# bio-phys/BioEM

Measured on AMD Instinct MI355X. Metric: image-comparisons/sec (orient×CTF×particle) at 224²; log P max-abs-diff vs CPU, higher is better.
Workload: dtype f32

## Files before the change

### bioem_amd/csrc/bioem_hip.hip

```cpp
#define BIOEM_MAIN_TU 1
#include "engine_types.hpp"

#include <rccl/rccl.h>

#include <dlfcn.h>

#include <map>
#include <memory>
#include <mutex>
#include <queue>
#include <string>
#include <vector>

namespace
{

struct HipErr
{
  std::string msg;
};

#define HIP_CHECK(h, expr)                                                                                         \
  do                                                                                                               \
  {                                                                                                                \
// ... 21 lines not shown
#include "compare_generic.hpp"
#include "compare_rows.hpp"
#include "compare_direct.hpp"
#include "kernel_select.hpp"
#include "fold_kernels.hpp"
#include "window_tiles.hpp"

struct bioem_hip_ctx
{
  int device = 0;
  hipStream_t stream = nullptr;
  PD pd;
  int nMaps = 0, nAngles = 0, nCTF = 0, algo = 1;
  int N = 0, H = 0, M = 0;
  int Hp = 0;
  size_t Mc = 0;
  KernelPlan plan;
  int pchunk = 128;
  int *dDispLocal = nullptr, *dTileCenter = nullptr, *dTileValid = nullptr, *dRankOfRow = nullptr;
  float *dBtab = nullptr;
  float2 *dConvShift = nullptr;
  Partial *dPartTiles = nullptr;
  int OB = 0;
  int maxOC = 0;
  int chunkB = 0;

  float2 *dRef = nullptr;
  float *dSumRef = nullptr, *dSumsqRef = nullptr;
  float2 *dCTF = nullptr;
  float *dCtfParam = nullptr;
  bioem_hip_model_point *dPts = nullptr;
  double *dStamp = nullptr;
  double modelRadius = 0.;
  double quatNormDev = 0.;
  int nPts = 0;
  float NormDen = 0, pixelSize = 0;
  int shiftX = 0, shiftY = 0;
  int iradMax = 0;
  bool direct = false;
  float *dMapsReal = nullptr, *dConvReal = nullptr;
  double2 *dDirectZ = nullptr;
  int nCU = 256;
  float4 *dAngles = nullptr;
  int nAnglesUp = 0, isQuat = 1;
  float2 *dTw = nullptr;
  double2 *dTwD = nullptr;
  int *dDisp = nullptr;
  double2 *dLtab = nullptr;
  float2 *dTwk = nullptr;
  float2 *dTwNyq = nullptr;
  float *dTnyq = nullptr;
  Partial *dPartials = nullptr;
  unsigned char *dProb = nullptr;
  size_t probBytes = 0;
  size_t devProbBytes = 0;
  bool shard = false;
  int angO0 = 0, angO1 = 0;
  bioem_hip_angle_candidate *dCand = nullptr;
  int candK = 0;
  unsigned char *dSend = nullptr, *dRecv = nullptr;
  size_t sendBytes = 0, recvBytes = 0;
  bioem_hip_prob_map *dMerged = nullptr;

  struct Slot
  {
    double *projReal = nullptr;
    double *tempDen = nullptr;
    double2 *rowSpec = nullptr;
    float2 *specRef = nullptr;
    float *scratch = nullptr;
    float2 *conv = nullptr;
    bioem_hip_param5 *params = nullptr;
    double2 *postc = nullptr;
    int stageO0 = 0, stageNO = 0, stageC0 = 0, stageNC = 0;
    hipEvent_t prepDone = nullptr, cmpDone = nullptr;
    bool cmpPending = false;
  };
  Slot slot[2];
  hipStream_t prepStream = nullptr;

  struct CompatHalf
  {
    float2 *hConv = nullptr;
    bioem_hip_param5 *hPar = nullptr;
    int2 *hIds = nullptr;
    int4 *hSeg = nullptr;
    float2 *dStage = nullptr;
    int2 *dIds = nullptr;
    int4 *dSeg = nullptr;
    hipEvent_t staged = nullptr;
  };
  CompatHalf ring[2];
  int ringCap = 0, ringHalf = 0, ringCount = 0;
  std::vector<int> ringOrients;
  hipStream_t copyStream = nullptr;

  struct Alloc
  {
    void *p;
    bool pinned;
  };
  std::vector<Alloc> allocs;

  struct PhaseEvents
  {
    int phase, o0, o1, c0, c1;
    hipEvent_t a, b;
  };
  bool phaseTiming = false;
  std::vector<PhaseEvents> phasePending;
  std::vector<bioem_hip_phase_record> phaseDone;
  std::vector<hipEvent_t> evPool;
  std::vector<std::pair<hipEvent_t, hipEvent_t>> evPending;
  double compareMs = 0;
  long long launches = 0, comparisons = 0;

  std::string err;
};

namespace
{

hipEvent_t get_event(bioem_hip_ctx *h)
{
  if (!h->evPool.empty())
  {
    hipEvent_t e = h->evPool.back();
    h->evPool.pop_back();
    return e;
  }
  hipEvent_t e;
  if (hipEventCreate(&e) != hipSuccess)
    return nullptr;
  return e;
}

void drain_events(bioem_hip_ctx *h)
{
  for (auto &pr : h->evPending)
  {
    float ms = 0.f;
    if (hipEventSynchronize(pr.second) == hipSuccess && hipEventElapsedTime(&ms, pr.first, pr.second) == hipSuccess)
      h->compareMs += (double) ms;
    h->evPool.push_back(pr.first);
    h->evPool.push_back(pr.second);
  }
  h->evPending.clear();
}

int phase_begin(bioem_hip_ctx *h, hipStream_t st, int phase, int o0, int o1, int c0, int c1)
{
  if (!h->phaseTiming)
    return 0;
  bioem_hip_ctx::PhaseEvents e = {phase, o0, o1, c0, c1, get_event(h), get_event(h)};
  if (!e.a || !e.b)
  {
    h->err = "hipEventCreate failed";
    return 1;
  }
  HIP_CHECK(h, hipEventRecord(e.a, st));
  h->phasePending.push_back(e);
  return 0;
}

int phase_end(bioem_hip_ctx *h, hipStream_t st)
{
  if (!h->phaseTiming || h->phasePending.empty())
    return 0;
  HIP_CHECK(h, hipEventRecord(h->phasePending.back().b, st));
  return 0;
}

void drain_phases(bioem_hip_ctx *h)
{
  for (auto &e : h->phasePending)
  {
    float ms = 0.f;
    if (hipEventSynchronize(e.b) == hipSuccess && hipEventElapsedTime(&ms, e.a, e.b) == hipSuccess)
    {
      bioem_hip_phase_record r = {e.phase, e.o0, e.o1, e.c0, e.c1, (double) ms * 1e-3};
      h->phaseDone.push_back(r);
    }
    h->evPool.push_back(e.a);
    h->evPool.push_back(e.b);
  }
  h->phasePending.clear();
}

template <class T>
int dev_alloc(bioem_hip_ctx *h, T *&p, size_t n)
{
  HIP_CHECK(h, hipMalloc(&p, sizeof(T) * n));
  if (p)
    h->allocs.push_back({p, false});
  return 0;
}
template <class T>
int host_alloc(bioem_hip_ctx *h, T *&p, size_t n)
{
  HIP_CHECK(h, hipHostMalloc(&p, sizeof(T) * n, hipHostMallocDefault));
  if (p)
    h->allocs.push_back({p, true});
  return 0;
}
template <class T>
void dev_release(bioem_hip_ctx *h, T *&p)
{
  if (!p)
    return;
  for (size_t i = 0; i < h->allocs.size(); i++)
    if (h->allocs[i].p == p)
    {
      h->allocs.erase(h->allocs.begin() + i);
      break;
    }
  hipFree(p);
  p = nullptr;
}
template <class T>
int upload(bioem_hip_ctx *h, T *&p, const T *src, size_t n)
{
  if (dev_alloc(h, p, n))
    return 1;
  HIP_CHECK(h, hipMemcpy(p, src, sizeof(T) * n, hipMemcpyHostToDevice));
  return 0;
}

double2 twiddle_d(long long ab, int N)
{
  const double ang = 2.0 * M_PI * (double) ((ab % N + N) % N) / (double) N;
  return make_double2(cos(ang), sin(ang));
}
float2 twiddle(long long ab, int N)
{
  const double2 w = twiddle_d(ab, N);
  return make_float2((float) w.x, (float) w.y);
}

void void_slot(bioem_hip_ctx::Slot &s) { s.stageNO = s.stageNC = 0; }

template <int Q>
void launch_nyquist_rows(bioem_hip_ctx *h, const CompareArgs &aw, int WD, int nOC)
{
  const int PB = 16 / Q;
  const dim3 gridq((unsigned) (((size_t) (h->nMaps + PB - 1) / PB) * ((nOC + 15) / 16)));
  switch (WD)
  {
#define X(W)                                                                                                            \
  case W:                                                                                                               \
    hipLaunchKernelGGL((k_nyquist_rows<W, Q>), gridq, dim3(256), 0, h->stream, aw);                                     \
    break;
    X(5) X(10) X(13) X(15) X(20) X(31) X(42)
#undef X
  }
}
void launch_nyquist(bioem_hip_ctx *h, const CompareArgs &aw, int WD, int nOC)
{
  if (h->nMaps <= 64)
    launch_nyquist_rows<4>(h, aw, WD, nOC);
  else
    launch_nyquist_rows<1>(h, aw, WD, nOC);
}

int launch_compare_fold(bioem_hip_ctx *h, const bioem_hip_ctx::Slot &bb, int nOC, int orient0, int conv0,
                        int convPerOrient, const int2 *ids = nullptr, const int4 *segs = nullptr, int nSeg = 0)
{
  const KernelPlan &P = h->plan;
  const int fam = P.family;
  CompareArgs a;
  a.ref = h->dRef;
  a.conv = bb.conv;
  a.params = bb.params;
  a.postc = bb.postc;
  a.sumRef = h->dSumRef;
  a.sumsqRef = h->dSumsqRef;
  a.tw = h->dTw;
  a.disp = h->dDisp;
  a.ltab = h->dLtab;
  a.twk = h->dTwk;
  a.btab = h->dBtab;
  a.tnyq = h->dTnyq;
  a.twnyq = h->dTwNyq;
  a.partials = h->dPartials;
  a.ldPart = h->maxOC;
  a.N = h->N;
  a.H = h->H;
  a.Hp = h->Hp;
  a.N1 = P.N1;
  a.nd = P.nd;
  a.maxD = h->pd.maxDisplaceCenter;
  a.nOC = nOC;
  a.nMaps = h->nMaps;
  a.algo = h->algo;
  a.pd = h->pd;
  a.gs = P.gs;
  a.ndx = a.ndy = P.nd;
  a.nyqWD = P.nyqWD;
  {
    const int cols = P.nyq ? h->H - 1 : h->H;
    const int nblkF = (cols + 63) / 64, rem = cols - (nblkF - 1) * 64;
    a.split = (fam == KF_FAST || fam == KF_FASTM) && rem <= 32 && P.N1 >= 2 &&
              (P.nyq || !getenv("BIOEM_NO_SPLIT_LAST"));
  }
  a.pchunk = h->pchunk > 0 ? std::min(h->pchunk, h->nMaps) : h->nMaps;
  if (a.pchunk >= 8)
    a.pchunk &= ~7;
  const int ocGroups = (nOC + 3) / 4;
  const bool groupPerXcd = h->nMaps <= 64 && (fam == KF_FAST || fam == KF_FASTM || fam == KF_FASTM2);
  if (groupPerXcd)
    a.pchunk = -1;
  dim3 grid((unsigned) ((size_t) (groupPerXcd ? (ocGroups + 7) / 8 * 8 : ocGroups) * h->nMaps)), block(256);
  if (fam == KF_WIDE2)
  {
    a.ts = P.w2TS;
    grid = dim3((unsigned) ((size_t) nOC * h->nMaps));
    block = dim3(64 * P.w2NW);
  }
  else if (fam == KF_GENERIC)
  {
    a.ts = P.genericRows;
    grid = dim3((unsigned) ((size_t) ((nOC + P.genericWaves - 1) / P.genericWaves) * h->nMaps));
    block = dim3(64 * P.genericWaves);
  }
  auto launch = [&](const CompareArgs &aw) {
    if (P.nyq)
      launch_nyquist(h, aw, P.nyqWD, nOC);
    hipLaunchKernelGGL(P.fn, grid, block, P.ldsBytes, h->stream, aw);
  };
  hipEvent_t e0 = get_event(h), e1 = get_event(h);
  if (!e0 || !e1)
  {
    if (e0)
      h->evPool.push_back(e0);
    if (e1)
      h->evPool.push_back(e1);
    h->err = "hipEventCreate failed";
    return 1;
  }
  hipLaunchKernelGGL(k_posterior_consts, dim3((nOC + 63) / 64), dim3(64), 0, h->stream, bb.params, h->pd, bb.postc, nOC);
  HIP_CHECK(h, hipEventRecord(e0, h->stream));
  if (phase_begin(h, h->stream, BIOEM_HIP_PHASE_COMPARISON, ids ? -1 : orient0, ids ? -1 : orient0 + (nOC + convPerOrient - 1) / convPerOrient,
                  ids ? -1 : conv0, ids ? -1 : conv0 + convPerOrient))
    return 1;
  if (h->direct)
  {
    CompareArgs ad = a;
    ad.gs = h->pd.GridSpaceCenter;
    ad.maxD = h->pd.maxDisplaceCenter;
    hipLaunchKernelGGL(k_c2r_cols, dim3(h->H, nOC), dim3(128), sizeof(double2) * h->N, h->stream, bb.conv, h->N, h->H,
                       P.halfR, P.N1, h->dTwD, h->dDirectZ);
    hipLaunchKernelGGL(k_c2r_rows, dim3(h->N, nOC), dim3(128), sizeof(double2) * h->H, h->stream, h->dDirectZ, h->N,
                       h->H, h->dTwD, h->dConvReal);
    const dim3 gridd((unsigned) ((size_t) nOC * ((h->nMaps + 31) / 32)));
    hipLaunchKernelGGL((k_compare_direct<3, 8>), gridd, dim3(512), direct_lds_bytes(h->N), h->stream, ad, h->dConvReal,
                       h->dMapsReal);
  }
  else if (!P.tileT)
    launch(a);
  else
  {
    const int nT = P.tilesPerAxis;
    const size_t tileStride = (size_t) h->nMaps * h->maxOC;
    const size_t total = (size_t) nOC * h->M;
    CompareArgs at = a;
    at.disp = h->dDispLocal;
    at.nd = P.tileT;
    at.maxD = P.winD * P.gs;
    for (int tx = 0; tx < nT; tx++)
      for (int ty = 0; ty < nT; ty++)
      {
        const int sx = P.gs * P.tileCenter[tx], sy = P.gs * P.tileCenter[ty];
        if (sx == 0 && sy == 0)
          at.conv = bb.conv;
        else
        {
          hipLaunchKernelGGL(k_phase_shift, dim3(2048), dim3(256), 0, h->stream, bb.conv, h->dConvShift, total, h->N,
                             h->H, P.halfR, P.N1, sx, sy, h->dTw);
          at.conv = h->dConvShift;
        }
        at.ndx = P.tileValid[tx];
        at.ndy = P.tileValid[ty];
        at.partials = h->dPartTiles + (size_t) (tx * nT + ty) * tileStride;
        launch(at);
      }
    const long long nt = (long long) nOC * h->nMaps;
    hipLaunchKernelGGL(k_merge_tiles, dim3((unsigned) ((nt + 255) / 256)), dim3(256), 0, h->stream, h->dPartTiles,
                       nT * nT, tileStride, h->maxOC, nOC, h->nMaps, P.tileT, nT, h->dTileCenter,
                       h->pd.maxDisplaceCenter / P.gs, P.nd, h->dRankOfRow, h->dPartials);
  }
  HIP_CHECK(h, hipGetLastError());
  HIP_CHECK(h, hipEventRecord(e1, h->stream));
  h->evPending.push_back({e0, e1});
  h->launches++;
  h->comparisons += (long long) nOC * h->nMaps;
  bioem_hip_prob_map *pmap = reinterpret_cast<bioem_hip_prob_map *>(h->dProb);
  bioem_hip_prob_angle *pang = reinterpret_cast<bioem_hip_prob_angle *>(h->dProb + sizeof(bioem_hip_prob_map) * h->nMaps);
  if (h->pd.writeAngles)
  {
    const int nRuns = ids ? nSeg : (nOC + convPerOrient - 1) / convPerOrient;
    const long long nt = (long long) nRuns * h->nMaps;
    hipLaunchKernelGGL(k_fold_angles, dim3((unsigned) ((nt + 255) / 256)), dim3(256), 0, h->stream, h->dPartials,
                       h->maxOC, nOC, h->nMaps, orient0, convPerOrient, segs, nRuns, pang, h->angO0);
  }
  if (h->nMaps <= 64 && nOC >= 1024)
    hipLaunchKernelGGL(k_fold_wave<4>, dim3(h->nMaps), dim3(256), 0, h->stream, h->dPartials, h->maxOC, nOC, h->nMaps,
                       bb.params, h->dSumRef, h->dDisp, P.nd, h->pd, orient0, conv0, convPerOrient, ids, pmap);
  else
    hipLaunchKernelGGL(k_fold_wave<1>, dim3((h->nMaps + 3) / 4), dim3(256), 0, h->stream, h->dPartials, h->maxOC, nOC,
                       h->nMaps, bb.params, h->dSumRef, h->dDisp, P.nd, h->pd, orient0, conv0, convPerOrient, ids,
                       pmap);
  HIP_CHECK(h, hipGetLastError());
  if (phase_end(h, h->stream))
    return 1;
  if (h->evPending.size() > 512)
    drain_events(h);
  return 0;
}

const int kMaxPixels = 5120;
constexpr int kDftTwLds = 3072;
size_t dft_rows_lds(int N) { return sizeof(double) * ((N <= kDftTwLds ? 5 : 3) * (size_t) N + 2); }
size_t dft_cols_lds(int N) { return sizeof(double2) * (N <= kDftTwLds ? 3 : 2) * (size_t) N; }
void dft_split(int N, int &A, int &B)
{
  A = 1;
  for (int d = 1; d * d <= N; d++)
    if (N % d == 0)
      A = d;
  B = N / A;
}
bool r2c_use_fft(int N)
{
  const char *e = getenv("BIOEM_R2C");
  return bioem_r2c_fft_supported(N) && !(e && !strcmp(e, "dft"));
}
bool dft_use_mfma(int N)
{
  int A, B;
  dft_split(N, A, B);
  return dft_mfma_fits(N, A, B);
}
hipError_t dft_allow_lds(int N)
{
  hipError_t e;
  if (dft_use_mfma(N))
  {
    const void *fns[4] = {reinterpret_cast<const void *>(k_dft_rows_mfma<2>),
                          reinterpret_cast<const void *>(k_dft_rows_mfma<kDftMfmaTiles>),
                          reinterpret_cast<const void *>(k_dft_cols_mfma<2>),
                          reinterpret_cast<const void *>(k_dft_cols_mfma<kDftMfmaTiles>)};
    for (int f = 0; f < 4; f++)
    {
      e = hipFuncSetAttribute(fns[f], hipFuncAttributeMaxDynamicSharedMemorySize,
                              (int) (f < 2 ? dft_mfma_rows_lds(N) : dft_mfma_cols_lds(N)));
      if (e != hipSuccess)
        return e;
    }
    return hipSuccess;
  }
  if (N <= kDftTwLds)
  {
    e = hipFuncSetAttribute(reinterpret_cast<const void *>(k_dft_rows<true>), hipFuncAttributeMaxDynamicSharedMemorySize,
                            (int) dft_rows_lds(N));
    if (e != hipSuccess)
      return e;
    return hipFuncSetAttribute(reinterpret_cast<const void *>(k_dft_cols<true>), hipFuncAttributeMaxDynamicSharedMemorySize,
                               (int) dft_cols_lds(N));
  }
  e = hipFuncSetAttribute(reinterpret_cast<const void *>(k_dft_rows<false>), hipFuncAttributeMaxDynamicSharedMemorySize,
                          (int) dft_rows_lds(N));
  if (e != hipSuccess)
    return e;
  return hipFuncSetAttribute(reinterpret_cast<const void *>(k_dft_cols<false>), hipFuncAttributeMaxDynamicSharedMemorySize,
                             (int) dft_cols_lds(N));
}

hipError_t conv_allow_lds()
{
  const void *fns[3] = {reinterpret_cast<const void *>(k_convolve_sums<3, 6>), reinterpret_cast<const void *>(k_convolve_sums<3, 5>),
                        reinterpret_cast<const void *>(k_convolve_sums<4, 4>)};
  for (const void *f : fns)
  {
    const hipError_t e = hipFuncSetAttribute(f, hipFuncAttributeMaxDynamicSharedMemorySize, (int) conv_lanes_lds(kLaneRows));
    if (e != hipSuccess)
      return e;
  }
  return hipSuccess;
}

hipError_t launch_r2c(hipStream_t st, int nCU, const double *srcD, const float *srcF, const double *tempDen, float NormDen,
                      int N, int nImg, const double2 *tw, double2 *rowSpec, float2 *out, int lo = 0, int side = 0)
{
  side = side ? side : N;
  const int H = N / 2 + 1;
  int A, B;
  dft_split(N, A, B);
  if (r2c_use_fft(N))
    return bioem_r2c_fft_launch(st, nCU, srcD, srcF, tempDen, NormDen, N, nImg, tw, rowSpec, out, lo, side);
  if (dft_use_mfma(N))
  {
    const int perCU = std::max(1, std::min(4, (int) (160 * 1024 / (dft_mfma_cols_lds(N) + 1024))));
    const int rowUnits = ((N + 15) / 16) * nImg, colUnits = ((H + 15) / 16) * nImg;
    if (A * ((B + 15) / 16) <= 2 * kDftMfmaWaves)
    {
      hipLaunchKernelGGL(k_dft_rows_mfma<2>, dim3(std::min(rowUnits, perCU * nCU)), dim3(kDftMfmaThreads),
                         dft_mfma_rows_lds(N), st, srcD, srcF, tempDen, NormDen, N, H, A, B, nImg, tw, rowSpec);
      hipLaunchKernelGGL(k_dft_cols_mfma<2>, dim3(std::min(colUnits, perCU * nCU)), dim3(kDftMfmaThreads),
                         dft_mfma_cols_lds(N), st, rowSpec, N, H, A, B, nImg, tw, out);
    }
    else
    {
      hipLaunchKernelGGL(k_dft_rows_mfma<kDftMfmaTiles>, dim3(std::min(rowUnits, nCU)), dim3(kDftMfmaThreads),
                         dft_mfma_rows_lds(N), st, srcD, srcF, tempDen, NormDen, N, H, A, B, nImg, tw, rowSpec);
      hipLaunchKernelGGL(k_dft_cols_mfma<kDftMfmaTiles>, dim3(std::min(colUnits, nCU)), dim3(kDftMfmaThreads),
                         dft_mfma_cols_lds(N), st, rowSpec, N, H, A, B, nImg, tw, out);
    }
  }
  else if (N <= kDftTwLds)
  {
    hipLaunchKernelGGL(k_dft_rows<true>, dim3(N, nImg), dim3(128), dft_rows_lds(N), st, srcD, srcF, tempDen, NormDen, N,
                       H, A, B, tw, rowSpec);
    hipLaunchKernelGGL(k_dft_cols<true>, dim3(H, nImg), dim3(256), dft_cols_lds(N), st, rowSpec, N, H, A, B, tw, out);
  }
  else
  {
    hipLaunchKernelGGL(k_dft_rows<false>, dim3(N, nImg), dim3(128), dft_rows_lds(N), st, srcD, srcF, tempDen, NormDen, N,
                       H, A, B, tw, rowSpec);
    hipLaunchKernelGGL(k_dft_cols<false>, dim3(H, nImg), dim3(256), dft_cols_lds(N), st, rowSpec, N, H, A, B, tw, out);
  }
  return hipGetLastError();
}

int run_r2c(bioem_hip_ctx *h, const bioem_hip_ctx::Slot &bb, hipStream_t st, const double *srcD, const float *srcF, int nImg,
            int lo = 0, int side = 0)
{
  HIP_CHECK(h, launch_r2c(st, h->nCU, srcD, srcF, bb.tempDen, h->NormDen, h->N, nImg, h->dTwD, bb.rowSpec, bb.specRef, lo,
                          side));
  return 0;
}

int project_batch(bioem_hip_ctx *h, const bioem_hip_ctx::Slot &bb, hipStream_t st, int o0, int nO)
{
  const int N = h->N;
  const double reach = h->modelRadius / (double) h->pixelSize;
  const int boxLo = std::max(0, (int) std::floor(N / 2.0 + 0.5 - reach) - 1 - h->iradMax - std::max(0, std::max(h->shiftX, h->shiftY)));
  const int boxHi = std::min(N - 1, (int) std::floor(N / 2.0 + 0.5 + reach) + 1 + h->iradMax - std::min(0, std::min(h->shiftX, h->shiftY)));
  const int boxSide = boxHi - boxLo + 1;
  const bool keepLength = h->quatNormDev * 4.0 * std::max(1.0, reach) < 0.5;
  if (h->dStamp && boxSide >= 1 && (size_t) boxSide * boxSide * sizeof(double) <= 52 * 1024 && N < 32768 &&
      keepLength)
  {
    const int compact = r2c_use_fft(N);
    hipLaunchKernelGGL(k_project_box, dim3(std::min(nO, 3 * h->nCU)), dim3(256), sizeof(double) * boxSide * boxSide, st,
                       h->dPts, h->nPts, h->dAngles, o0, h->isQuat, N, h->pixelSize, h->shiftX, h->shiftY, h->iradMax,
                       h->dStamp, boxLo, boxSide, nO, compact, bb.projReal, bb.tempDen);
    HIP_CHECK(h, hipGetLastError());
    return compact ? run_r2c(h, bb, st, bb.projReal, nullptr, nO, boxLo, boxSide) : run_r2c(h, bb, st, bb.projReal, nullptr, nO);
  }
  HIP_CHECK(h, hipMemsetAsync(bb.tempDen, 0, sizeof(double) * nO, st));
  const int TR = 40960 / (8 * N);
  const bool coordsFit = (size_t) h->nPts * sizeof(ProjectRecord) <= (size_t) N * h->H * sizeof(double2);
  if (TR >= 12 && h->iradMax <= 16 && h->dStamp && N < 32768 && coordsFit)
  {
    ProjectRecord *coords = reinterpret_cast<ProjectRecord *>(bb.rowSpec);
    hipLaunchKernelGGL(k_project_coords, dim3((h->nPts + 255) / 256, nO), dim3(256), 0, st, h->dPts, h->nPts, h->dAngles,
                       o0, h->isQuat, N, h->pixelSize, h->shiftX, h->shiftY, coords);
    const int units = ((N + TR - 1) / TR) * nO;
    hipLaunchKernelGGL(k_project_bands, dim3(std::min(units, 3 * h->nCU)), dim3(256), sizeof(double) * TR * N, st, coords,
                       h->nPts, nO, N, TR, h->iradMax, h->dStamp, bb.projReal, bb.tempDen);
  }
  else
  {
    HIP_CHECK(h, hipMemsetAsync(bb.projReal, 0, sizeof(double) * (size_t) nO * N * N, st));
    hipLaunchKernelGGL(k_project, dim3((h->nPts + 255) / 256, nO), dim3(256), 0, st, h->dPts, h->nPts, h->dAngles, o0,
                       h->isQuat, N, h->pixelSize, h->shiftX, h->shiftY, bb.projReal, bb.tempDen);
  }
  HIP_CHECK(h, hipGetLastError());
  return run_r2c(h, bb, st, bb.projReal, nullptr, nO);
}

int compat_alloc(bioem_hip_ctx *h)
{
  if (h->ringCap)
    return 0;
  int cap = 128;
  if (getenv("BIOEM_COMPAT_RING"))
    cap = atoi(getenv("BIOEM_COMPAT_RING"));
  cap = std::max(1, std::min(cap, h->maxOC));
  const size_t M = (size_t) h->M;
  for (int k = 0; k < 2; k++)
  {
    bioem_hip_ctx::CompatHalf &r = h->ring[k];
    if (host_alloc(h, r.hConv, M * cap) || host_alloc(h, r.hPar, cap) || host_alloc(h, r.hIds, cap) ||
        host_alloc(h, r.hSeg, cap) || dev_alloc(h, r.dStage, M * cap) || dev_alloc(h, r.dIds, cap) ||
        dev_alloc(h, r.dSeg, cap))
      return 1;
    HIP_CHECK(h, hipEventCreateWithFlags(&r.staged, hipEventDisableTiming));
  }
  HIP_CHECK(h, hipStreamCreateWithFlags(&h->copyStream, hipStreamNonBlocking));
  h->ringCap = cap;
  h->ringHalf = 0;
  h->ringCount = 0;
  return 0;
}

int compat_flush(bioem_hip_ctx *h)
{
  const int n = h->ringCount;
  if (n == 0)
    return 0;
  const int half = h->ringHalf;
  bioem_hip_ctx::CompatHalf &r = h->ring[half];
  bioem_hip_ctx::Slot &bb = h->slot[half];
  void_slot(bb);
// ... 1257 lines not shown
```

### bioem_amd/csrc/compare_args.hpp

```cpp
#ifndef BIOEM_COMPARE_ARGS_HPP
#define BIOEM_COMPARE_ARGS_HPP

namespace
{

struct CompareArgs
{
  const float2 *ref;
  const float2 *conv;
  const bioem_hip_param5 *params;
  const double2 *postc;
  const float *sumRef, *sumsqRef;
  const float2 *tw;
  const int *disp;
  const double2 *ltab;
  const float2 *twk;
  const float2 *twnyq;
  const float *btab;
  float *tnyq;
  Partial *partials;
  int ldPart;
  int N, H, N1, nd, maxD, nOC, nMaps, algo;
  int Hp;
  int pchunk;
  int gs;
  int ndx, ndy;
  int ts, nyqWD;
  int split;
  PD pd;
};

}

#endif
```

### bioem_amd/csrc/compare_fast.hpp

```cpp
#ifndef BIOEM_COMPARE_FAST_HPP
#define BIOEM_COMPARE_FAST_HPP

namespace
{

typedef const float2 __attribute__((address_space(4))) *const_float2_ptr;
__device__ __forceinline__ const_float2_ptr as_constant(const float2 *p)
{
  return (const_float2_ptr) (unsigned long long) p;
}

template <typename T>
__device__ __forceinline__ T *uniform_ptr(T *p)
{
  const unsigned long long v = (unsigned long long) p;
  const unsigned lo = __builtin_amdgcn_readfirstlane((unsigned) v);
  const unsigned hi = __builtin_amdgcn_readfirstlane((unsigned) (v >> 32));
  return (T *) (((unsigned long long) hi << 32) | lo);
}

__device__ __noinline__ double log_slow_path(float f) { return log((double) f); }

__device__ __forceinline__ double log_of_float(float f, const double2 *ltab)
{
  const unsigned int bits = __float_as_uint(f);
  if (!(f > 1.1754944e-38f) || bits >= 0x7f800000u)
    return log_slow_path(f);
  const int e = (int) (bits >> 23) - 127;
  const float m = __uint_as_float((bits & 0x007fffffu) | 0x3f800000u);
  const double2 t = ltab[(bits >> 17) & 63];
  const double r = fma((double) m, t.x, -1.0);
  double p = fma(r, -1.0 / 6.0, 1.0 / 5.0);
  p = fma(r, p, -1.0 / 4.0);
  p = fma(r, p, 1.0 / 3.0);
  p = fma(r, p, -1.0 / 2.0);
  p = fma(r * r, p, r);
  return fma((double) e, 0.693147180559945309417232, t.y + p);
}

__device__ __forceinline__ double exp_fast_nonpos(double x) { return (double) __expf((float) x); }

struct LseF
{
  float m;
  double s;
  int id;
  float val;
};

__device__ __forceinline__ void lsef_push(LseF &L, double lp, int id, float val, int algo)
{
  const float lpf = (float) lp;
  const double lpe = (algo == 1) ? (double) lpf : lp;
  if (L.m < lpf)
  {
    L.s = (L.m == -INFINITY) ? 0. : L.s * exp_fast_nonpos((double) L.m - (double) lpf);
    L.m = lpf;
    L.id = id;
    L.val = val;
  }
  else if (L.m == lpf && id < L.id)
  {
    L.id = id;
    L.val = val;
  }
  L.s += exp_fast_nonpos(lpe - (double) L.m);
}

__device__ __forceinline__ void lsef_wave_reduce(LseF &L)
{
  for (int off = 32; off > 0; off >>= 1)
  {
    const float m2 = __shfl_xor(L.m, off);
    const double s2 = __shfl_xor(L.s, off);
    const int id2 = __shfl_xor(L.id, off);
    const float v2 = __shfl_xor(L.val, off);
    if (m2 > L.m || (m2 == L.m && id2 < L.id))
    {
      const double sc = (L.m == -INFINITY) ? 0. : L.s * exp_fast_nonpos((double) L.m - (double) m2);
      L.s = sc + s2;
      L.m = m2;
      L.id = id2;
      L.val = v2;
    }
    else
    {
      const double sc = (m2 == -INFINITY) ? 0. : s2 * exp_fast_nonpos((double) m2 - (double) L.m);
      L.s += sc;
    }
  }
}

struct PostW
{
  float Np, nn, rnn;
  float k0, k1, k2, k3;
  double A, t2, prior;
};

__device__ __forceinline__ PostW post_consts(float Np, int N, const bioem_hip_param5 &q, float sumref, float sumsqref,
                                             double t2, double prior)
{
  PostW w;
  w.Np = Np;
  w.nn = (float) (N * N);
  w.rnn = 1.0f / w.nn;
  w.k0 = sumsqref * q.sumsquareC;
  w.k1 = 2 * sumref * q.sumC;
  w.k2 = sumsqref * q.sumC * q.sumC;
  w.k3 = sumref * sumref * q.sumsquareC;
  w.A = (double) (3 - Np) * 0.5;
  w.t2 = t2;
  w.prior = prior;
  return w;
}

__device__ __forceinline__ float div_by_nn(float a, const PostW &w)
{
  const float q = a * w.rnn;
  const float r = fmaf(-q, w.nn, a);
  return fmaf(r, w.rnn, q);
}

template <int B>
__device__ __forceinline__ void posterior_batch(LseF &L, const float (&acc)[B], const int (&id)[B], const bool (&ok)[B],
                                                const PostW &w, const double2 *ltab, int algo)
{
  float cc[B], fe[B];
  bool bad = false;
#pragma unroll
  for (int v = 0; v < B; v++)
  {
    cc[v] = div_by_nn(acc[v], w);
    const float f = w.Np * (w.k0 - cc[v] * cc[v]) + w.k1 * cc[v] - w.k2 - w.k3;
    fe[v] = ok[v] ? f : 1.f;
    bad = bad || !(fe[v] > 1.1754944e-38f) || __float_as_uint(fe[v]) >= 0x7f800000u;
  }
  double lg[B];
  if (__builtin_expect(__any(bad), 0))
  {
#pragma unroll
    for (int v = 0; v < B; v++)
      lg[v] = log_of_float(fe[v], ltab);
  }
  else
  {
    double2 t[B];
#pragma unroll
    for (int v = 0; v < B; v++)
      t[v] = ltab[(__float_as_uint(fe[v]) >> 17) & 63];
#pragma unroll
    for (int v = 0; v < B; v++)
    {
      const unsigned int bits = __float_as_uint(fe[v]);
      const int e = (int) (bits >> 23) - 127;
      const float m = __uint_as_float((bits & 0x007fffffu) | 0x3f800000u);
      const double r = fma((double) m, t[v].x, -1.0);
      double p = fma(r, -1.0 / 6.0, 1.0 / 5.0);
      p = fma(r, p, -1.0 / 4.0);
      p = fma(r, p, 1.0 / 3.0);
      p = fma(r, p, -1.0 / 2.0);
      p = fma(r * r, p, r);
      lg[v] = fma((double) e, 0.693147180559945309417232, t[v].y + p);
    }
  }
  float lpf[B];
  double lpe[B];
#pragma unroll
  for (int v = 0; v < B; v++)
  {
    double lp = w.A * lg[v] + w.t2;
    lp -= w.prior;
    lpf[v] = ok[v] ? (float) lp : -INFINITY;
    lpe[v] = (algo == 1) ? (double) lpf[v] : lp;
  }
  float mb = lpf[0], vb = cc[0];
  int ib = ok[0] ? id[0] : 0x7fffffff;
#pragma unroll
  for (int v = 1; v < B; v++)
  {
    const bool t = ok[v] && (lpf[v] > mb || (lpf[v] == mb && id[v] < ib));
    mb = t ? lpf[v] : mb;
    ib = t ? id[v] : ib;
    vb = t ? cc[v] : vb;
  }
  const bool take = mb > L.m || (mb == L.m && ib < L.id);
  const float newm = fmaxf(L.m, mb);
  double sum = (L.m == newm) ? L.s : L.s * exp_fast_nonpos((double) L.m - (double) newm);
#pragma unroll
  for (int v = 0; v < B; v++)
  {
    const double e = exp_fast_nonpos(lpe[v] - (double) newm);
    sum += ok[v] ? e : 0.;
  }
  L.s = sum;
  L.m = newm;
  L.id = take ? ib : L.id;
  L.val = take ? vb : L.val;
}

__device__ __forceinline__ bool fast_block_pair(const CompareArgs &a, int &p, int &ocg)
{
  const int ocGroups = (a.nOC + 3) >> 2;
  if (a.pchunk < 0)
  {
    const int x = blockIdx.x & 7, q = blockIdx.x >> 3;
    ocg = (q / a.nMaps) * 8 + x;
    p = q % a.nMaps;
    return ocg < ocGroups;
  }
  const int per = a.pchunk * ocGroups;
  int c = blockIdx.x / per;
  const int nch = (a.nMaps + a.pchunk - 1) / a.pchunk;
  c = min(c, nch - 1);
  const int rem = blockIdx.x - c * per;
  const int pc = min(a.pchunk, a.nMaps - c * a.pchunk);
  ocg = rem / pc;
  p = c * a.pchunk + (rem - ocg * pc);
  return true;
}

template <int NR, bool STATIC, int NP, int TS>
__device__ __forceinline__ void window_accumulate(const float2 *Tl, const float2 *twl, int N, int step, int idx0,
                                                  const int (&rowoff)[NR], int nr, float (&acc)[NR], int npairs = NP)
{
  int idx = idx0;
#pragma unroll 2
  for (int kp = 0; kp < npairs; kp++)
  {
    const float2 w0 = twl[idx];
    idx += step;
    if (idx >= N)
      idx -= N;
    const float2 w1 = twl[idx];
    idx += step;
    if (idx >= N)
      idx -= N;
#pragma unroll
    for (int r = 0; r < NR; r++)
    {
      if (STATIC || r < nr)
      {
        const float4 t = *reinterpret_cast<const float4 *>(&Tl[(STATIC ? rowoff[0] + r * TS : rowoff[r]) + 2 * kp]);
        float v = acc[r];
        v = fmaf(t.x, w0.x, v);
        v = fmaf(-t.y, w0.y, v);
        v = fmaf(t.z, w1.x, v);
        v = fmaf(-t.w, w1.y, v);
        acc[r] = v;
      }
    }
  }
}

#define FFT_IN(k) (is_pow2(R) ? bitrevR<R>(k) : DIGITREV<R>.pos[k])
#define FFT_OUT(n) (n)
#define FFT_RUN(xr, xi)                                                                                            \
  do                                                                                                               \
  {                                                                                                                \
    if constexpr (is_pow2(R))                                                                                      \
      fft_inverse_dit<R>(xr, xi);                                                                                  \
    else                                                                                                           \
      fft_inverse_mixed<R>(xr, xi);                                                                                \
  } while (0)
template <int WD, int R, bool NYQ, int GS>
__global__ __launch_bounds__(256, 3) void k_compare_fast(const CompareArgs a)
{
  static_assert(WD <= 10, "windows of at most 21 rows; 27 / 31 rows: k_compare_fastm");
  constexpr int NW = 2 * WD + 1;
  constexpr int R2 = R / 2;
  constexpr int RD = (R2 % 4 == 0) ? 4 : (R2 == 15) ? 3 : (R2 % 5 == 0) ? 5 : (R2 % 3 == 0) ? 3 : (R2 % 2 == 0) ? 2 : 1;
  constexpr int NR = (WD <= 5) ? 3 : 7;
  constexpr int TS = 66;
  extern __shared__ __align__(16) unsigned char smem[];
  const int N = a.N, H = a.H, N1 = a.N1;
  float2 *twl = reinterpret_cast<float2 *>(smem);
  int *displ = reinterpret_cast<int *>(smem + (size_t) ((N + 2) & ~1) * 8);
  double2 *ltab = reinterpret_cast<double2 *>(smem + (size_t) ((N + 2) & ~1) * 8 + 256);
  float2 *Tall = reinterpret_cast<float2 *>(smem + (size_t) ((N + 2) & ~1) * 8 + 256 + 1024);
  const int wave = __builtin_amdgcn_readfirstlane((int) (threadIdx.x >> 6));
  const int lane = threadIdx.x & 63;
  float2 *Tl = Tall + (size_t) wave * NW * TS;

  for (int t = threadIdx.x; t <= N; t += blockDim.x)
    twl[t] = a.tw[t];
  int *dinv = displ + 32;
  const int mD = a.maxD / GS;
  for (int t = threadIdx.x; t < a.nd; t += blockDim.x)
  {
    const int dv = a.disp[t];
    displ[t] = dv;
    const int m = dv / GS + mD;
    if (m >= 0 && m < 32)
      dinv[m] = t;
  }
  for (int t = threadIdx.x; t < 64; t += blockDim.x)
    ltab[t] = a.ltab[t];
  __syncthreads();

  int p, ocg;
  if (!fast_block_pair(a, p, ocg))
    return;
  const int oc_raw = ocg * 4 + wave;
  const bool oc_valid = oc_raw < a.nOC;
  const int oc = oc_valid ? oc_raw : a.nOC - 1;
  const int Hp = a.Hp;
  const size_t M = (size_t) N * Hp;
  const auto rsrcF = __builtin_amdgcn_make_buffer_rsrc(uniform_ptr(const_cast<float2 *>(a.ref + (size_t) p * M)), 0,
                                                       (int) (M * sizeof(float2)), 0x00020000);
  const auto rsrcC = __builtin_amdgcn_make_buffer_rsrc(uniform_ptr(const_cast<float2 *>(a.conv + (size_t) oc * M)), 0,
                                                       (int) (M * sizeof(float2)), 0x00020000);

  const int nd = a.nd;
  const int G = 64 / nd;
  const int nr = (nd + G - 1) / G;
  const int iy = lane % nd, grp = lane / nd;
  const bool wactive = grp < G;
  const int dy = displ[iy];
  const int step = dy < 0 ? dy + N : dy;
  const bool is_static = (nr == NR) && (nd == G * NR) && (nd == 2 * mD + 1);
  float acc[NR];
#pragma unroll
  for (int r = 0; r < NR; r++)
    acc[r] = 0.f;
  auto row_of = [&](int r) -> int {
    int ix = wactive ? grp * nr + r : r;
    if (ix >= nd)
      ix = nd - 1;
    return (displ[ix] / GS + WD) * TS;
  };
  const int rowbase = is_static ? ((wactive ? grp : 0) * NR - mD + WD) * TS : row_of(0);

  const int nblk = NYQ ? (H - 1 + 63) / 64 : (H + 63) / 64;
  const unsigned rowbytes = (unsigned) Hp * 16u;
  constexpr bool SPLIT_OK = !(NYQ && R == 32);
  const int sHalf = (N1 + 1) >> 1;
  const int hsel = lane >> 5;
  const unsigned halfoff = (unsigned) (hsel * sHalf * R2) * rowbytes;
  auto lane_offset = [&](int b) -> unsigned {
    const bool sp = SPLIT_OK && a.split && b == nblk - 1;
    const int kyb = b * 64 + (sp ? (lane & 31) : lane);
    return (unsigned) (kyb < H ? kyb : H - 1) * 16u + (sp ? halfoff : 0u);
  };
  u32x4 rf[RD], rc[RD];
  {
    const unsigned lo0 = lane_offset(0);
#pragma unroll
    for (int t = 0; t < RD; t++)
    {
      rf[t] = __builtin_amdgcn_raw_buffer_load_b128(rsrcF, lo0, (unsigned) t * rowbytes, 0);
      rc[t] = __builtin_amdgcn_raw_buffer_load_b128(rsrcC, lo0, (unsigned) t * rowbytes, 0);
    }
  }
  for (int blk = 0; blk < nblk; blk++)
  {
    const bool split = SPLIT_OK && a.split && blk == nblk - 1;
    const int n1 = split ? sHalf : N1;
    const int ttotal = R2 * n1;
    const int ky = blk * 64 + (split ? (lane & 31) : lane);
    const unsigned laneoff = lane_offset(blk);
    const unsigned laneoff_next = lane_offset(min(blk + 1, nblk - 1));
    const bool has_next = blk + 1 < nblk;
    float Tr[NW], Ti[NW];
#pragma unroll
    for (int d = 0; d < NW; d++)
    {
      Tr[d] = 0.f;
      Ti[d] = 0.f;
    }
    if (ky < H)
    for (int k1 = 0; k1 < n1; k1++)
    {
      float xr[R], xi[R];
      float2 wk[NW];
      const float2 *twk = a.twk + (size_t) k1 * NW;
#pragma unroll
      for (int d = 0; d < NW; d++)
        wk[d] = twk[d];
#pragma unroll
      for (int k2p = 0; k2p < R2; k2p++)
      {
        const float4 f = as_float4(rf[k2p % RD]);
        const float4 c = as_float4(rc[k2p % RD]);
        xr[FFT_IN(2 * k2p)] = fmaf(c.x, f.x, c.y * f.y);
        xi[FFT_IN(2 * k2p)] = fmaf(c.y, f.x, -(c.x * f.y));
        xr[FFT_IN(2 * k2p + 1)] = fmaf(c.z, f.z, c.w * f.w);
        xi[FFT_IN(2 * k2p + 1)] = fmaf(c.w, f.z, -(c.z * f.w));
        int tn = k1 * R2 + k2p + RD;
        unsigned vo = laneoff;
        if (k2p + RD >= R2 && tn >= ttotal)
        {
          tn = has_next ? tn - ttotal : ttotal - 1;
          vo = has_next ? laneoff_next : laneoff;
        }
        rf[k2p % RD] = __builtin_amdgcn_raw_buffer_load_b128(rsrcF, vo, (unsigned) tn * rowbytes, 0);
        rc[k2p % RD] = __builtin_amdgcn_raw_buffer_load_b128(rsrcC, vo, (unsigned) tn * rowbytes, 0);
        __builtin_amdgcn_sched_barrier(0);
      }
      FFT_RUN(xr, xi);
#pragma unroll
      for (int d = -WD; d <= WD; d++)
      {
        const int pos = FFT_OUT((((d * GS) % R) + R) % R);
        const float2 w = wk[d + WD];
        float tr = Tr[d + WD], ti = Ti[d + WD];
        tr = fmaf(xr[pos], w.x, tr);
        tr = fmaf(-xi[pos], w.y, tr);
        ti = fmaf(xr[pos], w.y, ti);
        ti = fmaf(xi[pos], w.x, ti);
        Tr[d + WD] = tr;
        Ti[d + WD] = ti;
      }
    }
    if (split)
    {
      const float2 *ws = a.twk + (size_t) sHalf * NW;
#pragma unroll
      for (int d = 0; d < NW; d++)
      {
        const float2 w = ws[d];
        const float wx = hsel ? w.x : 1.f, wy = hsel ? w.y : 0.f;
        const float tr = fmaf(-Ti[d], wy, Tr[d] * wx), ti = fmaf(Ti[d], wx, Tr[d] * wy);
        const u32x2 sr = __builtin_amdgcn_permlane32_swap(__float_as_uint(tr), __float_as_uint(tr), false, false);
        const u32x2 si = __builtin_amdgcn_permlane32_swap(__float_as_uint(ti), __float_as_uint(ti), false, false);
        Tr[d] = __uint_as_float(sr.x) + __uint_as_float(sr.y);
        Ti[d] = __uint_as_float(si.x) + __uint_as_float(si.y);
      }
    }
    float wgt = 2.f;
    if (ky == 0 || (((N & 1) == 0) && ky == N / 2))
      wgt = 1.f;
    if (ky >= H || (split && hsel))
      wgt = 0.f;
    {
      __syncthreads();
#pragma unroll
      for (int d = 0; d < NW; d++)
        Tl[d * TS + lane] = make_float2(Tr[d] * wgt, Ti[d] * wgt);
      __syncthreads();
      const int idx0 = (int) (((long long) (blk * 64) * step) % N);
      const int npairs = min(32, (H - blk * 64 + 1) >> 1);
      if (is_static)
      {
        const int rowoff[NR] = {rowbase};
        window_accumulate<NR, true, 32, TS>(Tl, twl, N, step, idx0, rowoff, nr, acc, npairs);
      }
      else
      {
        int rowoff[NR];
#pragma unroll
        for (int r = 0; r < NR; r++)
          rowoff[r] = row_of(r);
        window_accumulate<NR, false, 32, TS>(Tl, twl, N, step, idx0, rowoff, nr, acc, npairs);
      }
    }
  }
  if (NYQ)
  {
    const float *tq = a.tnyq + ((size_t) p * a.ldPart + oc) * NW;
    const float sg = (dy & 1) ? -1.f : 1.f;
#pragma unroll
    for (int r = 0; r < NR; r++)
      acc[r] = fmaf(sg, tq[is_static ? rowbase / TS + r : row_of(r) / TS], acc[r]);
  }

  const double2 pc = a.postc[oc];
  const PostW pw = post_consts(a.pd.Ntotpi, N, a.params[oc], a.sumRef[p], a.sumsqRef[p], pc.x, pc.y);
  LseF L;
  L.m = -INFINITY;
  L.s = 0.;
  L.id = 0x7fffffff;
  L.val = 0.f;
  {
    constexpr int PB = NR > 8 ? 8 : NR;
#pragma unroll
    for (int r0 = 0; r0 < NR; r0 += PB)
    {
      float accv[PB];
      int idv[PB];
      bool okv[PB];
#pragma unroll
      for (int j = 0; j < PB; j++)
      {
        const int r = r0 + j < NR ? r0 + j : NR - 1;
        const int ixs = grp * nr + r;
        okv[j] = r0 + j < NR && r < nr && wactive && ixs < a.ndx && iy < a.ndy;
        const int ix = is_static ? dinv[min(ixs, 31)] : ixs;
        accv[j] = acc[r];
        idv[j] = ix * nd + iy;
      }
      posterior_batch<PB>(L, accv, idv, okv, pw, ltab, a.algo);
    }
  }
  lsef_wave_reduce(L);
  if (lane == 0 && oc_valid)
  {
    Partial r;
    r.sumExp = L.s;
    r.best = L.m;
    r.id = L.id;
    r.value = L.val;
    r.pad = 0;
    a.partials[(size_t) p * a.ldPart + oc] = r;
  }
}

template <int WD, int Q>
__global__ __launch_bounds__(256) void k_nyquist_rows(const CompareArgs a)
{
  static_assert(Q == 1 || Q == 4, "one thread per pair, or one per pair and wave");
  constexpr int NW = 2 * WD + 1;
  __shared__ float part[Q == 4 ? 2 * 64 * NW : 1];
  const int N = a.N, H = a.H, N1 = a.N1;
  const int R2 = N / (2 * N1);
  const int tilesOC = (a.nOC + 15) / 16;
  const int tp = blockIdx.x / tilesOC, to = blockIdx.x - tp * tilesOC;
  const int q = Q == 1 ? 0 : __builtin_amdgcn_readfirstlane((int) (threadIdx.x >> 6));
  const int t = Q == 1 ? threadIdx.x : threadIdx.x & 63;
  const int p = tp * (16 / Q) + (t >> 4), oc = to * 16 + (t & 15);
  const bool valid = p < a.nMaps && oc < a.nOC;
  const size_t M = (size_t) N * a.Hp;
  const float2 *F = a.ref + (size_t) (valid ? p : 0) * M;
  const float2 *C = a.conv + (size_t) (valid ? oc : 0) * M;
  float acc[NW];
#pragma unroll
  for (int d = 0; d < NW; d++)
    acc[d] = 0.f;
  const int nRP = N1 * R2 / Q;
  constexpr int NB = WD > 31 ? 4 : 8;
  for (int rp0 = q * nRP; rp0 < (q + 1) * nRP; rp0 += NB)
  {
    float4 cb[NB], fb[NB];
#pragma unroll
    for (int u = 0; u < NB; u++)
    {
      const size_t li = ((size_t) (rp0 + u) * a.Hp + N / 2) * 2;
      cb[u] = *reinterpret_cast<const float4 *>(C + li);
      fb[u] = *reinterpret_cast<const float4 *>(F + li);
    }
#pragma unroll
    for (int u = 0; u < NB; u++)
    {
      const float4 c = cb[u], f = fb[u];
      const float x0r = fmaf(c.x, f.x, c.y * f.y), x0i = fmaf(c.y, f.x, -(c.x * f.y));
      const float x1r = fmaf(c.z, f.z, c.w * f.w), x1i = fmaf(c.w, f.z, -(c.z * f.w));
      const float4 *tw = reinterpret_cast<const float4 *>(a.twnyq + (size_t) (rp0 + u) * NW * 2);
#pragma unroll
      for (int d = 0; d < NW; d++)
      {
        const float4 w = tw[d];
        float v = acc[d];
        v = fmaf(x0r, w.x, v);
        v = fmaf(-x0i, w.y, v);
        v = fmaf(x1r, w.z, v);
        v = fmaf(-x1i, w.w, v);
        acc[d] = v;
      }
    }
  }
  if (Q == 4)
  {
    float *mine = part + ((q >> 1) * 64 + t) * NW;
    if (q & 1)
    {
#pragma unroll
      for (int d = 0; d < NW; d++)
        mine[d] = acc[d];
    }
    __syncthreads();
    if (!(q & 1))
    {
#pragma unroll
      for (int d = 0; d < NW; d++)
        acc[d] += mine[d];
    }
    __syncthreads();
    if (q == 2)
    {
#pragma unroll
      for (int d = 0; d < NW; d++)
        mine[d] = acc[d];
    }
    __syncthreads();
    if (q == 0)
    {
#pragma unroll
      for (int d = 0; d < NW; d++)
        acc[d] += part[(64 + t) * NW + d];
    }
  }
  if (valid && q == 0)
  {
    float *o = a.tnyq + ((size_t) p * a.ldPart + oc) * NW;
#pragma unroll
    for (int d = 0; d < NW; d++)
      o[d] = acc[d];
  }
}

}

#endif
```

Baseline: 54.33 million.

## Process two particle maps per block in fast compare kernel to reuse conv loads

For one specific configuration (window 10, radix 16, no Nyquist, grid step 1), each block of k_compare_fast now handles two reference maps at once. It loads each convolved-map tile once and reuses it across both particles, and the grid shrinks to match. This cuts the global loads of the conv data and the twiddle setup per comparison. In exchange it roughly doubles register use (launch bounds lowered to two blocks per CU) and doubles the LDS window-accumulate passes per block, which may reduce occupancy.

```diff
diff --git a/bioem_amd/csrc/bioem_hip.hip b/bioem_amd/csrc/bioem_hip.hip
--- a/bioem_amd/csrc/bioem_hip.hip
+++ b/bioem_amd/csrc/bioem_hip.hip
@@ -347,14 +347,16 @@
     a.split = (fam == KF_FAST || fam == KF_FASTM) && rem <= 32 && P.N1 >= 2 &&
               (P.nyq || !getenv("BIOEM_NO_SPLIT_LAST"));
   }
-  a.pchunk = h->pchunk > 0 ? std::min(h->pchunk, h->nMaps) : h->nMaps;
+  const int pairs = fam == KF_FAST ? fast_pairs(P.winD, 2 * P.halfR, P.nyq, P.gs) : 1;
+  const int units = (h->nMaps + pairs - 1) / pairs;
+  a.pchunk = h->pchunk > 0 ? std::min(std::max(h->pchunk / pairs, 1), units) : units;
   if (a.pchunk >= 8)
     a.pchunk &= ~7;
   const int ocGroups = (nOC + 3) / 4;
   const bool groupPerXcd = h->nMaps <= 64 && (fam == KF_FAST || fam == KF_FASTM || fam == KF_FASTM2);
   if (groupPerXcd)
     a.pchunk = -1;
-  dim3 grid((unsigned) ((size_t) (groupPerXcd ? (ocGroups + 7) / 8 * 8 : ocGroups) * h->nMaps)), block(256);
+  dim3 grid((unsigned) ((size_t) (groupPerXcd ? (ocGroups + 7) / 8 * 8 : ocGroups) * units)), block(256);
   if (fam == KF_WIDE2)
   {
     a.ts = P.w2TS;
diff --git a/bioem_amd/csrc/compare_args.hpp b/bioem_amd/csrc/compare_args.hpp
--- a/bioem_amd/csrc/compare_args.hpp
+++ b/bioem_amd/csrc/compare_args.hpp
@@ -30,6 +30,8 @@
   PD pd;
 };
 
+constexpr int fast_pairs(int WD, int R, bool NYQ, int GS) { return (WD == 10 && R == 16 && !NYQ && GS == 1) ? 2 : 1; }
+
 }
 
 #endif
diff --git a/bioem_amd/csrc/compare_fast.hpp b/bioem_amd/csrc/compare_fast.hpp
--- a/bioem_amd/csrc/compare_fast.hpp
+++ b/bioem_amd/csrc/compare_fast.hpp
@@ -199,22 +199,23 @@
   L.val = take ? vb : L.val;
 }
 
-__device__ __forceinline__ bool fast_block_pair(const CompareArgs &a, int &p, int &ocg)
+__device__ __forceinline__ bool fast_block_pair(const CompareArgs &a, int &p, int &ocg, int PP = 1)
 {
   const int ocGroups = (a.nOC + 3) >> 2;
+  const int nU = (a.nMaps + PP - 1) / PP;
   if (a.pchunk < 0)
   {
     const int x = blockIdx.x & 7, q = blockIdx.x >> 3;
-    ocg = (q / a.nMaps) * 8 + x;
-    p = q % a.nMaps;
+    ocg = (q / nU) * 8 + x;
+    p = q % nU;
     return ocg < ocGroups;
   }
   const int per = a.pchunk * ocGroups;
   int c = blockIdx.x / per;
-  const int nch = (a.nMaps + a.pchunk - 1) / a.pchunk;
+  const int nch = (nU + a.pchunk - 1) / a.pchunk;
   c = min(c, nch - 1);
   const int rem = blockIdx.x - c * per;
-  const int pc = min(a.pchunk, a.nMaps - c * a.pchunk);
+  const int pc = min(a.pchunk, nU - c * a.pchunk);
   ocg = rem / pc;
   p = c * a.pchunk + (rem - ocg * pc);
   return true;
@@ -264,9 +265,10 @@
       fft_inverse_mixed<R>(xr, xi);                                                                                \
   } while (0)
 template <int WD, int R, bool NYQ, int GS>
-__global__ __launch_bounds__(256, 3) void k_compare_fast(const CompareArgs a)
+__global__ __launch_bounds__(256, fast_pairs(WD, R, NYQ, GS) == 2 ? 2 : 3) void k_compare_fast(const CompareArgs a)
 {
   static_assert(WD <= 10, "windows of at most 21 rows; 27 / 31 rows: k_compare_fastm");
+  constexpr int PP = fast_pairs(WD, R, NYQ, GS);
   constexpr int NW = 2 * WD + 1;
   constexpr int R2 = R / 2;
   constexpr int RD = (R2 % 4 == 0) ? 4 : (R2 == 15) ? 3 : (R2 % 5 == 0) ? 5 : (R2 % 3 == 0) ? 3 : (R2 % 2 == 0) ? 2 : 1;
@@ -298,16 +300,27 @@
     ltab[t] = a.ltab[t];
   __syncthreads();
 
-  int p, ocg;
-  if (!fast_block_pair(a, p, ocg))
+  int pu, ocg;
+  if (!fast_block_pair(a, pu, ocg, PP))
     return;
   const int oc_raw = ocg * 4 + wave;
   const bool oc_valid = oc_raw < a.nOC;
   const int oc = oc_valid ? oc_raw : a.nOC - 1;
+  int p[PP];
+  bool p_valid[PP];
+#pragma unroll
+  for (int j = 0; j < PP; j++)
+  {
+    p_valid[j] = PP == 1 || pu * PP + j < a.nMaps;
+    p[j] = p_valid[j] ? pu * PP + j : a.nMaps - 1;
+  }
   const int Hp = a.Hp;
   const size_t M = (size_t) N * Hp;
-  const auto rsrcF = __builtin_amdgcn_make_buffer_rsrc(uniform_ptr(const_cast<float2 *>(a.ref + (size_t) p * M)), 0,
-                                                       (int) (M * sizeof(float2)), 0x00020000);
+  __amdgpu_buffer_rsrc_t rsrcF[PP];
+#pragma unroll
+  for (int j = 0; j < PP; j++)
+    rsrcF[j] = __builtin_amdgcn_make_buffer_rsrc(uniform_ptr(const_cast<float2 *>(a.ref + (size_t) p[j] * M)), 0,
+                                                 (int) (M * sizeof(float2)), 0x00020000);
   const auto rsrcC = __builtin_amdgcn_make_buffer_rsrc(uniform_ptr(const_cast<float2 *>(a.conv + (size_t) oc * M)), 0,
                                                        (int) (M * sizeof(float2)), 0x00020000);
 
@@ -319,10 +332,12 @@
   const int dy = displ[iy];
   const int step = dy < 0 ? dy + N : dy;
   const bool is_static = (nr == NR) && (nd == G * NR) && (nd == 2 * mD + 1);
-  float acc[NR];
-#pragma unroll
-  for (int r = 0; r < NR; r++)
-    acc[r] = 0.f;
+  float acc[PP][NR];
+#pragma unroll
+  for (int j = 0; j < PP; j++)
+#pragma unroll
+    for (int r = 0; r < NR; r++)
+      acc[j][r] = 0.f;
   auto row_of = [&](int r) -> int {
     int ix = wactive ? grp * nr + r : r;
     if (ix >= nd)
@@ -342,13 +357,15 @@
     const int kyb = b * 64 + (sp ? (lane & 31) : lane);
     return (unsigned) (kyb < H ? kyb : H - 1) * 16u + (sp ? halfoff : 0u);
   };
-  u32x4 rf[RD], rc[RD];
+  u32x4 rf[PP][RD], rc[RD];
   {
     const unsigned lo0 = lane_offset(0);
 #pragma unroll
     for (int t = 0; t < RD; t++)
     {
-      rf[t] = __builtin_amdgcn_raw_buffer_load_b128(rsrcF, lo0, (unsigned) t * rowbytes, 0);
+#pragma unroll
+      for (int j = 0; j < PP; j++)
+        rf[j][t] = __builtin_amdgcn_raw_buffer_load_b128(rsrcF[j], lo0, (unsigned) t * rowbytes, 0);
       rc[t] = __builtin_amdgcn_raw_buffer_load_b128(rsrcC, lo0, (unsigned) t * rowbytes, 0);
     }
   }
@@ -361,17 +378,19 @@
     const unsigned laneoff = lane_offset(blk);
     const unsigned laneoff_next = lane_offset(min(blk + 1, nblk - 1));
     const bool has_next = blk + 1 < nblk;
-    float Tr[NW], Ti[NW];
-#pragma unroll
-    for (int d = 0; d < NW; d++)
-    {
-      Tr[d] = 0.f;
-      Ti[d] = 0.f;
-    }
+    float Tr[PP][NW], Ti[PP][NW];
+#pragma unroll
+    for (int j = 0; j < PP; j++)
+#pragma unroll
+      for (int d = 0; d < NW; d++)
+      {
+        Tr[j][d] = 0.f;
+        Ti[j][d] = 0.f;
+      }
     if (ky < H)
     for (int k1 = 0; k1 < n1; k1++)
     {
-      float xr[R], xi[R];
+      float xr[PP][R], xi[PP][R];
       float2 wk[NW];
       const float2 *twk = a.twk + (size_t) k1 * NW;
 #pragma unroll
@@ -380,12 +399,16 @@
 #pragma unroll
       for (int k2p = 0; k2p < R2; k2p++)
       {
-        const float4 f = as_float4(rf[k2p % RD]);
         const float4 c = as_float4(rc[k2p % RD]);
-        xr[FFT_IN(2 * k2p)] = fmaf(c.x, f.x, c.y * f.y);
-        xi[FFT_IN(2 * k2p)] = fmaf(c.y, f.x, -(c.x * f.y));
-        xr[FFT_IN(2 * k2p + 1)] = fmaf(c.z, f.z, c.w * f.w);
-        xi[FFT_IN(2 * k2p + 1)] = fmaf(c.w, f.z, -(c.z * f.w));
+#pragma unroll
+        for (int j = 0; j < PP; j++)
+        {
+          const float4 f = as_float4(rf[j][k2p % RD]);
+          xr[j][FFT_IN(2 * k2p)] = fmaf(c.x, f.x, c.y * f.y);
+          xi[j][FFT_IN(2 * k2p)] = fmaf(c.y, f.x, -(c.x * f.y));
+          xr[j][FFT_IN(2 * k2p + 1)] = fmaf(c.z, f.z, c.w * f.w);
+          xi[j][FFT_IN(2 * k2p + 1)] = fmaf(c.w, f.z, -(c.z * f.w));
+        }
         int tn = k1 * R2 + k2p + RD;
         unsigned vo = laneoff;
         if (k2p + RD >= R2 && tn >= ttotal)
@@ -393,23 +416,31 @@
           tn = has_next ? tn - ttotal : ttotal - 1;
           vo = has_next ? laneoff_next : laneoff;
         }
-        rf[k2p % RD] = __builtin_amdgcn_raw_buffer_load_b128(rsrcF, vo, (unsigned) tn * rowbytes, 0);
+#pragma unroll
+        for (int j = 0; j < PP; j++)
+          rf[j][k2p % RD] = __builtin_amdgcn_raw_buffer_load_b128(rsrcF[j], vo, (unsigned) tn * rowbytes, 0);
         rc[k2p % RD] = __builtin_amdgcn_raw_buffer_load_b128(rsrcC, vo, (unsigned) tn * rowbytes, 0);
         __builtin_amdgcn_sched_barrier(0);
       }
-      FFT_RUN(xr, xi);
+#pragma unroll
+      for (int j = 0; j < PP; j++)
+        FFT_RUN(xr[j], xi[j]);
 #pragma unroll
       for (int d = -WD; d <= WD; d++)
       {
         const int pos = FFT_OUT((((d * GS) % R) + R) % R);
         const float2 w = wk[d + WD];
-        float tr = Tr[d + WD], ti = Ti[d + WD];
-        tr = fmaf(xr[pos], w.x, tr);
-        tr = fmaf(-xi[pos], w.y, tr);
-        ti = fmaf(xr[pos], w.y, ti);
-        ti = fmaf(xi[pos], w.x, ti);
-        Tr[d + WD] = tr;
-        Ti[d + WD] = ti;
+#pragma unroll
+        for (int j = 0; j < PP; j++)
+        {
+          float tr = Tr[j][d + WD], ti = Ti[j][d + WD];
+          tr = fmaf(xr[j][pos], w.x, tr);
+          tr = fmaf(-xi[j][pos], w.y, tr);
+          ti = fmaf(xr[j][pos], w.y, ti);
+          ti = fmaf(xi[j][pos], w.x, ti);
+          Tr[j][d + WD] = tr;
+          Ti[j][d + WD] = ti;
+        }
       }
     }
     if (split)
@@ -420,11 +451,15 @@
       {
         const float2 w = ws[d];
         const float wx = hsel ? w.x : 1.f, wy = hsel ? w.y : 0.f;
-        const float tr = fmaf(-Ti[d], wy, Tr[d] * wx), ti = fmaf(Ti[d], wx, Tr[d] * wy);
-        const u32x2 sr = __builtin_amdgcn_permlane32_swap(__float_as_uint(tr), __float_as_uint(tr), false, false);
-        const u32x2 si = __builtin_amdgcn_permlane32_swap(__float_as_uint(ti), __float_as_uint(ti), false, false);
-        Tr[d] = __uint_as_float(sr.x) + __uint_as_float(sr.y);
-        Ti[d] = __uint_as_float(si.x) + __uint_as_float(si.y);
+#pragma unroll
+        for (int j = 0; j < PP; j++)
+        {
+          const float tr = fmaf(-Ti[j][d], wy, Tr[j][d] * wx), ti = fmaf(Ti[j][d], wx, Tr[j][d] * wy);
+          const u32x2 sr = __builtin_amdgcn_permlane32_swap(__float_as_uint(tr), __float_as_uint(tr), false, false);
+          const u32x2 si = __builtin_amdgcn_permlane32_swap(__float_as_uint(ti), __float_as_uint(ti), false, false);
+          Tr[j][d] = __uint_as_float(sr.x) + __uint_as_float(sr.y);
+          Ti[j][d] = __uint_as_float(si.x) + __uint_as_float(si.y);
+        }
       }
     }
     float wgt = 2.f;
@@ -432,18 +467,20 @@
       wgt = 1.f;
     if (ky >= H || (split && hsel))
       wgt = 0.f;
+#pragma unroll
+    for (int j = 0; j < PP; j++)
     {
       __syncthreads();
 #pragma unroll
       for (int d = 0; d < NW; d++)
-        Tl[d * TS + lane] = make_float2(Tr[d] * wgt, Ti[d] * wgt);
+        Tl[d * TS + lane] = make_float2(Tr[j][d] * wgt, Ti[j][d] * wgt);
       __syncthreads();
       const int idx0 = (int) (((long long) (blk * 64) * step) % N);
       const int npairs = min(32, (H - blk * 64 + 1) >> 1);
       if (is_static)
       {
         const int rowoff[NR] = {rowbase};
-        window_accumulate<NR, true, 32, TS>(Tl, twl, N, step, idx0, rowoff, nr, acc, npairs);
+        window_accumulate<NR, true, 32, TS>(Tl, twl, N, step, idx0, rowoff, nr, acc[j], npairs);
       }
       else
       {
@@ -451,57 +488,65 @@
 #pragma unroll
         for (int r = 0; r < NR; r++)
           rowoff[r] = row_of(r);
-        window_accumulate<NR, false, 32, TS>(Tl, twl, N, step, idx0, rowoff, nr, acc, npairs);
+        window_accumulate<NR, false, 32, TS>(Tl, twl, N, step, idx0, rowoff, nr, acc[j], npairs);
       }
     }
   }
   if (NYQ)
   {
-    const float *tq = a.tnyq + ((size_t) p * a.ldPart + oc) * NW;
     const float sg = (dy & 1) ? -1.f : 1.f;
 #pragma unroll
-    for (int r = 0; r < NR; r++)
-      acc[r] = fmaf(sg, tq[is_static ? rowbase / TS + r : row_of(r) / TS], acc[r]);
+    for (int j = 0; j < PP; j++)
+    {
+      const float *tq = a.tnyq + ((size_t) p[j] * a.ldPart + oc) * NW;
+#pragma unroll
+      for (int r = 0; r < NR; r++)
+        acc[j][r] = fmaf(sg, tq[is_static ? rowbase / TS + r : row_of(r) / TS], acc[j][r]);
+    }
   }
 
   const double2 pc = a.postc[oc];
-  const PostW pw = post_consts(a.pd.Ntotpi, N, a.params[oc], a.sumRef[p], a.sumsqRef[p], pc.x, pc.y);
-  LseF L;
-  L.m = -INFINITY;
-  L.s = 0.;
-  L.id = 0x7fffffff;
-  L.val = 0.f;
-  {
-    constexpr int PB = NR > 8 ? 8 : NR;
-#pragma unroll
-    for (int r0 = 0; r0 < NR; r0 += PB)
-    {
-      float accv[PB];
-      int idv[PB];
-      bool okv[PB];
-#pragma unroll
-      for (int j = 0; j < PB; j++)
-      {
-        const int r = r0 + j < NR ? r0 + j : NR - 1;
-        const int ixs = grp * nr + r;
-        okv[j] = r0 + j < NR && r < nr && wactive && ixs < a.ndx && iy < a.ndy;
-        const int ix = is_static ? dinv[min(ixs, 31)] : ixs;
-        accv[j] = acc[r];
-        idv[j] = ix * nd + iy;
-      }
-      posterior_batch<PB>(L, accv, idv, okv, pw, ltab, a.algo);
-    }
-  }
-  lsef_wave_reduce(L);
-  if (lane == 0 && oc_valid)
-  {
-    Partial r;
-    r.sumExp = L.s;
-    r.best = L.m;
-    r.id = L.id;
-    r.value = L.val;
-    r.pad = 0;
-    a.partials[(size_t) p * a.ldPart + oc] = r;
+#pragma unroll
+  for (int j = 0; j < PP; j++)
+  {
+    const PostW pw = post_consts(a.pd.Ntotpi, N, a.params[oc], a.sumRef[p[j]], a.sumsqRef[p[j]], pc.x, pc.y);
+    LseF L;
+    L.m = -INFINITY;
+    L.s = 0.;
+    L.id = 0x7fffffff;
+    L.val = 0.f;
+    {
+      constexpr int PB = NR > 8 ? 8 : NR;
+#pragma unroll
+      for (int r0 = 0; r0 < NR; r0 += PB)
+      {
+        float accv[PB];
+        int idv[PB];
+        bool okv[PB];
+#pragma unroll
+        for (int v = 0; v < PB; v++)
+        {
+          const int r = r0 + v < NR ? r0 + v : NR - 1;
+          const int ixs = grp * nr + r;
+          okv[v] = r0 + v < NR && r < nr && wactive && ixs < a.ndx && iy < a.ndy;
+          const int ix = is_static ? dinv[min(ixs, 31)] : ixs;
+          accv[v] = acc[j][r];
+          idv[v] = ix * nd + iy;
+        }
+        posterior_batch<PB>(L, accv, idv, okv, pw, ltab, a.algo);
+      }
+    }
+    lsef_wave_reduce(L);
+    if (lane == 0 && oc_valid && p_valid[j])
+    {
+      Partial r;
+      r.sumExp = L.s;
+      r.best = L.m;
+      r.id = L.id;
+      r.value = L.val;
+      r.pad = 0;
+      a.partials[(size_t) p[j] * a.ldPart + oc] = r;
+    }
   }
 }
 
```

New measurement: 55.58 million (median of 6 runs). 1.02x the previous value.
